# fdrmrc/fictitious_domain_AL_preconditioners

Measured on AMD Instinct MI355X. Metric: FGMRES iterations/sec to 1e-8 residual, 3D Stokes-immersed (AL-preconditioned), higher is better.
Workload: dtype f64

## Files before the change

### fictitious_domain_al_preconditioners_amd/csrc/alfd.hip

```cpp

#include <hip/hip_runtime.h>
#include <rccl/rccl.h>

#include <algorithm>
#include <atomic>
#include <chrono>
#include <cmath>
#include <cstdio>
#include <cstdlib>
#include <cstring>
#include <memory>
#include <climits>
#include <condition_variable>
#include <functional>
#include <mutex>
#include <string>
#include <thread>
#include <unordered_set>
#include <vector>

#include "alfd/alfd.h"
#include "kernels.hpp"
#include "kernels_vs.hpp"

// ... 91 lines not shown
  std::vector<int64_t> rp;
  std::vector<int32_t> col;
  std::vector<double> val;
  int64_t nnz() const { return rp.empty() ? 0 : rp.back(); }
};

constexpr int kScratchSlot = ALFD_NSLOTS;

struct MlLevel {
  DevCsr A, C, Ct;
  DevCsr P, R;
  int64_t n = 0, npad = 0;
  double *dinv = nullptr;
  double lmax = 0;
  double *r = nullptr, *z = nullptr, *t = nullptr, *cd = nullptr, *cres = nullptr, *ctmp = nullptr;
  DevCsr gA, gC, gCt, gP, gR;
  bool P_global_cols = false;
  int64_t gn = 0, gnpad = 0, g_maxpiece = 0;
  std::vector<int64_t> g_offs;
  double *gdinv = nullptr, *gr = nullptr, *gz = nullptr, *gt = nullptr, *gcd = nullptr, *gcres = nullptr,
         *gctmp = nullptr, *g_send = nullptr, *g_stage = nullptr;
};

enum State { ITERATE = 0, SUCCESS = 1, FAILURE = 2 };
struct Control {
  alfd_control c;
  double initial = 0, reduced_tol = 0, last_value = 0;
  int last_step = 0;
  State check(int step, double v) {
    last_step = step;
// ... 58 lines not shown
  double *n_sc = nullptr, *n_sc_host = nullptr, *n_partial = nullptr, *n_gather = nullptr;
  int64_t mass_its = 0;
  HostCsr h_M, h_K;
  std::vector<int32_t> ml_agg[ALFD_MAX_LEVELS];
  std::vector<double> ml_wgt[ALFD_MAX_LEVELS];
  int64_t ml_ncoarse[ALFD_MAX_LEVELS] = {0, 0, 0, 0, 0, 0, 0, 0};
  HostCsr ml_P[ALFD_MAX_LEVELS];
  DevCsr ml_inv;
  struct Patch {
    bool on = false;
    int64_t m = 0, mpad = 0;
    DevCsr Ass, As, Ats, Cs, Cts;
    int32_t *S = nullptr;
    double *dinv = nullptr, *rS = nullptr, *zS = nullptr, *uS = nullptr, *eS = nullptr, *cd = nullptr,
           *cres = nullptr, *ctmp = nullptr, *rr = nullptr;
    double lmax = 0;
    bool rep = false;
    int64_t m_loc = 0, piece = 1, lam_piece = 1;
    std::vector<int64_t> soff;
    DevCsr Cts_loc, Ctg;
    double *send = nullptr, *stage = nullptr, *lam_send = nullptr, *lam_stage = nullptr, *loc = nullptr;
  } patch;
  std::vector<MlLevel> ml;
  int ml_rep_level = -1;
  bool dots_replicated = false;
  int64_t ml_rep_threshold = 300000;
  int ml_gpu_galerkin = 1;
  double *g_w = nullptr, *g_tlam = nullptr;
  std::vector<int64_t> ml_coff[ALFD_MAX_LEVELS];
  const int64_t *up_col_offsets = nullptr;
// ... 14 lines not shown
  double lambda_max = 0, lambda_min = 0;
  int64_t inner_its = 0, mp_its = 0;
  int inner_failures = 0, precond_applications = 0;
  std::vector<double> history;
  int timing = 0;
  std::vector<TimedLaunch> timed;
  double t_ms[ALFD_T_NCLASSES] = {0, 0, 0, 0};
  int64_t t_launches[ALFD_T_NCLASSES] = {0, 0, 0, 0};
  double t_bytes[ALFD_T_NCLASSES] = {0, 0, 0, 0};
  double t_fbytes[ALFD_T_NCLASSES] = {0, 0, 0, 0};
  double setup_s[ALFD_SETUP_NPHASES] = {0, 0, 0, 0, 0, 0, 0, 0};
  bool upload_since_setup = false;
  std::vector<void *> allocs;
  int spmv_stream_R = 2, spmv_stream_U = 8, spmv_nt = 0, spmv_grid_mult = 8;
  int spmv_group_R = 4, spmv_group_U = 4;
  bool vi_off = false;
  int vi_rows_R = 4, vi_rows_J = 2;
  int vi_xcd = 0;
  int vi_levels = 1;
  int vi_batched = 1;
  int win_RB_vi = 96;
  int win_vi = 1;
  int win_short_scale = 2;
  int vs_enable = 1, vs_NW = 4, vs_RB = 96, vs_xcd = 0, vs_share = 1, vs_wide = 1;
  int vs_lds_base_ok = -1;
  std::vector<int64_t> rb_ptr[ALFD_NSLOTS + 1];
  std::vector<int32_t> rb_rows[ALFD_NSLOTS + 1];
  int win_short_min_blocks = 256;
  int win_min_blocks = 256;
  int win_enable = 1, win_RB = 96, win_maxW = 4096, win_gap = 8, win_xcd = 0;
// ... 179 lines not shown
    hipEventElapsedTime(&ms, t.a, t.b);
    ctx->t_ms[t.cls] += ms;
    hipEventDestroy(t.a);
    hipEventDestroy(t.b);
  }
  ctx->timed.clear();
}

template <int L>
static void launch_spmv_L(alfd_ctx *ctx, const DevCsr &m, const double *x, double *y, int epi, double alpha,
                          const double *d, double *y2) {
  const int grid = grid_for_rows(m.n_list, L);
  const double *xh = m.halo;
#define ALFD_SPMV(EPI, SP)                                                                          \
  hipLaunchKernelGGL((spmv_kernel<L, EPI, SP>), dim3(grid), dim3(kBlock), 0, ctx->stream, m.n_list, \
                     m.rp, m.col, m.val, m.rows, x, xh, m.n_local_cols, y, alpha, d, y2)
  if (m.sparse) {
    if (epi == 0) ALFD_SPMV(0, true);
    else if (epi == 1) ALFD_SPMV(1, true);
    else if (epi == 2) ALFD_SPMV(2, true);
    else ALFD_SPMV(3, true);
  } else {
    if (epi == 0) ALFD_SPMV(0, false);
    else if (epi == 1) ALFD_SPMV(1, false);
    else if (epi == 2) ALFD_SPMV(2, false);
    else ALFD_SPMV(3, false);
  }
#undef ALFD_SPMV
}

template <int R, int U, bool NT>
static void launch_stream(alfd_ctx *ctx, const DevCsr &m, const double *x, double *y, int epi, double alpha,
                          const double *d, double *y2) {
  const int64_t nbatches = (m.nrows + R - 1) / R;
  const int grid = (int)std::max<int64_t>(1, std::min<int64_t>((nbatches + 3) / 4, 256 * ctx->spmv_grid_mult));
#define ALFD_STREAM(EPI)                                                                              \
  hipLaunchKernelGGL((spmv_stream_kernel<R, U, EPI, NT>), dim3(grid), dim3(kBlock), 0, ctx->stream,   \
                     m.nrows, m.rp, m.col, m.val, x, m.halo, m.n_local_cols, y, alpha, d, y2)
  if (epi == 0) ALFD_STREAM(0);
  else if (epi == 1) ALFD_STREAM(1);
  else if (epi == 2) ALFD_STREAM(2);
  else ALFD_STREAM(3);
#undef ALFD_STREAM
}

template <bool NT>
static bool launch_stream_RU(alfd_ctx *ctx, const DevCsr &m, const double *x, double *y, int epi,
                             double alpha, const double *d, double *y2) {
  const int R = ctx->spmv_stream_R, U = ctx->spmv_stream_U;
#define ALFD_RU(RR, UU) \
  if (R == RR && U == UU) return launch_stream<RR, UU, NT>(ctx, m, x, y, epi, alpha, d, y2), true
  ALFD_RU(2, 2); ALFD_RU(2, 4); ALFD_RU(4, 2); ALFD_RU(4, 4); ALFD_RU(4, 8); ALFD_RU(8, 4); ALFD_RU(8, 8);
  ALFD_RU(1, 4); ALFD_RU(2, 8); ALFD_RU(8, 2);
#undef ALFD_RU
  return false;
}

// ... 111 lines not shown
  ALFD_RU(1, 4); ALFD_RU(2, 4); ALFD_RU(2, 8); ALFD_RU(4, 2); ALFD_RU(4, 4); ALFD_RU(4, 8); ALFD_RU(8, 4);
  ALFD_RU(1, 8); ALFD_RU(1, 16); ALFD_RU(2, 16);
#undef ALFD_RU
  return false;
}


template <int L>
static void launch_vss(alfd_ctx *ctx, const DevCsr &m, const double *x, double *y, int epi, double alpha,
                       const double *d, double *y2) {
  const DevCsr::Vs &v = m.vs;
  const size_t lds = (size_t)kVsWinOff + (size_t)v.maxW * sizeof(double);
#define ALFD_VSS(EPI, TAG)                                                                                          \
  hipLaunchKernelGGL((spmv_vss_kernel<L, EPI, TAG>), dim3((unsigned)v.nb), dim3(256), lds, ctx->stream, v.stream, \
                     v.sb, v.tab, v.cnt, v.stride, v.seg_begin, v.blkW, v.seg_col, v.seg_off, v.doff, v.dn, v.dict, \
                     x, m.halo, m.n_local_cols, y, alpha, d, y2)
  if (m.tag == 0) {
    if (epi == 0) ALFD_VSS(0, 0);
    else if (epi == 1) ALFD_VSS(1, 0);
    else if (epi == 2) ALFD_VSS(2, 0);
    else ALFD_VSS(3, 0);
  } else {
    if (epi == 0) ALFD_VSS(0, 1);
    else if (epi == 1) ALFD_VSS(1, 1);
    else if (epi == 2) ALFD_VSS(2, 1);
    else ALFD_VSS(3, 1);
  }
#undef ALFD_VSS
}

static bool launch_vs(alfd_ctx *ctx, const DevCsr &m, const double *x, double *y, int epi, double alpha,
                      const double *d, double *y2, int64_t first_block = 0, int64_t n_blocks = -1) {
  const DevCsr::Vs &v = m.vs;
  if (ctx->vs_lds_base_ok < 0) {
    uint32_t *probe = nullptr, base = 1;
    if (hipMalloc((void **)&probe, sizeof(uint32_t)) == hipSuccess) {
      hipLaunchKernelGGL(vs_lds_base_probe_kernel, dim3(1), dim3(64), 4096, ctx->stream, probe);
      hipMemcpyAsync(&base, probe, sizeof(uint32_t), hipMemcpyDeviceToHost, ctx->stream);
      hipStreamSynchronize(ctx->stream);
      hipFree(probe);
// ... 35 lines not shown
  } while (0)
  if (NW == 8) ALFD_VS_E(8);
  else if (NW == 2) ALFD_VS_E(2);
  else ALFD_VS_E(4);
#undef ALFD_VS_E
#undef ALFD_VS
#undef ALFD_VS_ARGS
  return true;
}

static int halo_exchange(alfd_ctx *ctx, DevCsr &m, const double *x, hipStream_t st = nullptr);
static int spmv_launch_local(alfd_ctx *ctx, DevCsr &m, const double *x, double *y, int epi, double alpha, const double *d,
                             double *y2);

static int spmv_m(alfd_ctx *ctx, DevCsr &m, int cls, const double *x, double *y, int epi, double alpha = 0.0,
                  const double *d = nullptr, double *y2 = nullptr) {
  if (!m.present) return ctx->err = "matrix not set", ALFD_E_NOT_SETUP;
  const bool exchange = ctx->nranks > 1 && !m.rep && (ctx->local || ctx->host_alltoallv || m.n_halo > 0 || m.send_off.back() > 0);
  const bool overlap = exchange && (ctx->overlap_halo > 0 || (ctx->overlap_halo < 0 && (ctx->local || ctx->host_alltoallv))) && ctx->xstream && m.vs.on && m.vs.L == 64 && ctx->vs_enable && !ctx->vi_off &&
                       m.vs.nb_interior > 0 && !m.sparse && m.n_list > 0;
  if (overlap) {
    Timer tm(ctx, cls, m.algorithmic_bytes(), m.streamed_bytes(true, true));
    HIPC(hipEventRecord(ctx->ev_x, ctx->stream));
    if (!launch_vs(ctx, m, x, y, epi, alpha, d, y2, 0, m.vs.nb_interior)) return ctx->err = "batch-major launch failed", ALFD_E_HIP;
    HIPC(hipStreamWaitEvent(ctx->xstream, ctx->ev_x, 0));
    RC(halo_exchange(ctx, m, x, ctx->xstream));
    HIPC(hipEventRecord(ctx->ev_halo, ctx->xstream));
    HIPC(hipStreamWaitEvent(ctx->stream, ctx->ev_halo, 0));
    launch_vs(ctx, m, x, y, epi, alpha, d, y2, m.vs.nb_interior, m.vs.nb - m.vs.nb_interior);
    HIPC(hipGetLastError());
    return ALFD_OK;
  }
  if (exchange) RC(halo_exchange(ctx, m, x));
  if (m.sparse && epi != 1) {
    HIPC(hipMemsetAsync(y, 0, m.nrows * sizeof(double), ctx->stream));
    if (epi == 3) HIPC(hipMemsetAsync(y2, 0, m.nrows * sizeof(double), ctx->stream));
  }
  if (m.n_list == 0) return ALFD_OK;
  Timer tm(ctx, cls, m.algorithmic_bytes(), m.streamed_bytes(!ctx->vi_off, ctx->vs_enable != 0 && !ctx->vi_off));
  return spmv_launch_local(ctx, m, x, y, epi, alpha, d, y2);
}

static int spmv_launch_local(alfd_ctx *ctx, DevCsr &m, const double *x, double *y, int epi, double alpha, const double *d,
                             double *y2) {
  if (m.vs.on && ctx->vs_enable && !ctx->vi_off && launch_vs(ctx, m, x, y, epi, alpha, d, y2)) {
    HIPC(hipGetLastError());
    return ALFD_OK;
  }
  if (m.win && launch_window_RU(ctx, m, x, y, epi, alpha, d, y2)) {
    HIPC(hipGetLastError());
    return ALFD_OK;
  }
  if (m.L == 64 && !m.sparse && ctx->spmv_stream_R > 0) {
    const bool ok = ctx->spmv_nt ? launch_stream_RU<true>(ctx, m, x, y, epi, alpha, d, y2)
                                 : launch_stream_RU<false>(ctx, m, x, y, epi, alpha, d, y2);
    if (ok) {
      HIPC(hipGetLastError());
      return ALFD_OK;
    }
  }
  switch (m.L) {
    case 4: launch_spmv_L<4>(ctx, m, x, y, epi, alpha, d, y2); break;
    case 8: launch_spmv_L<8>(ctx, m, x, y, epi, alpha, d, y2); break;
    case 16: launch_spmv_L<16>(ctx, m, x, y, epi, alpha, d, y2); break;
    case 32: launch_spmv_L<32>(ctx, m, x, y, epi, alpha, d, y2); break;
    default: launch_spmv_L<64>(ctx, m, x, y, epi, alpha, d, y2); break;
  }
  HIPC(hipGetLastError());
  return ALFD_OK;
}

static int pick_short_row_format(alfd_ctx *ctx, DevCsr &m) {
  if (!m.vs.on || m.vs.L == 64 || m.nnz < 20000000 || ctx->vi_off || !ctx->vs_enable || m.sparse) return ALFD_OK;
  double *x = nullptr, *y = nullptr;
  const int64_t nx = std::max<int64_t>(ctx->nranks > 1 && !m.rep ? m.n_local_cols : m.ncols, 1);
  HIPC(hipMalloc((void **)&x, nx * sizeof(double)));
  HIPC(hipMalloc((void **)&y, std::max<int64_t>(m.nrows, 1) * sizeof(double)));
  HIPC(hipMemsetAsync(x, 0, nx * sizeof(double), ctx->stream));
  hipEvent_t e0, e1;
  HIPC(hipEventCreate(&e0));
  HIPC(hipEventCreate(&e1));
  float t[2] = {0.f, 0.f};
  bool ok = true;
  for (int f = 0; f < 2 && ok; ++f) {
// ... 2385 lines not shown

static int upload_matrix(alfd_ctx *ctx, int slot, int64_t nrows, int64_t ncols, const int64_t *rp,
                         const int32_t *col, const double *val);
static int upload_level(alfd_ctx *ctx, DevCsr &dst, const HostCsr &h) {
  static const int32_t no_col = 0;
  static const double no_val = 0;
  RC(upload_matrix(ctx, kScratchSlot, h.nrows, h.ncols, h.rp.data(), h.col.empty() ? &no_col : h.col.data(),
                   h.val.empty() ? &no_val : h.val.data()));
  csr_free(dst);
  dst = std::move(ctx->mat[kScratchSlot]);
  ctx->mat[kScratchSlot] = DevCsr();
  dst.tag = 1;
  return ALFD_OK;
}

static int level_op(alfd_ctx *ctx, int l, const double *x, double *y) {
  if (l == 0) return op_apply(ctx, OP_AUG, x, y);
  MlLevel &L = ctx->ml[l];
  RC(spmv_m(ctx, L.A, ALFD_T_SPMV_OTHER, x, y, 0));
  if (ctx->cfg.aug_assembled) return ALFD_OK;
  RC(spmv_m(ctx, L.C, ALFD_T_SPMV_OTHER, x, ctx->t_lam, 2, 0.0, ctx->diag[ALFD_INVW]));
  return spmv_m(ctx, L.Ct, ALFD_T_SPMV_OTHER, ctx->t_lam, y, 1, ctx->cfg.gamma);
}

static int level_cheb(alfd_ctx *ctx, int l, int degree, double ratio, const double *r, double *z) {
  MlLevel &L = ctx->ml[l];
  const double lmax = L.lmax, lmin = lmax / ratio;
  const double theta = 0.5 * (lmax + lmin), delta = 0.5 * (lmax - lmin);
  const double sigma = theta / delta;
  double rho = 1.0 / sigma;
  VEC_LAUNCH(cheb_init_kernel, L.npad, degree > 1 ? 40 : 32, 1.0 / theta, L.dinv, r, L.cd, z, L.cres,
             degree > 1 ? 1 : 0);
  for (int j = 1; j < degree; ++j) {
    RC(level_op(ctx, l, L.cd, L.ctmp));
    const double rho_new = 1.0 / (2.0 * sigma - rho);
    const double c1 = rho_new * rho, c2 = 2.0 * rho_new / delta;
    VEC_LAUNCH(cheb_step_kernel, L.npad, 64, c1, c2, L.dinv, L.ctmp, L.cres, L.cd, z);
    rho = rho_new;
  }
  HIPC(hipGetLastError());
  return ALFD_OK;
}

static int level_op_rep(alfd_ctx *ctx, int l, const double *x, double *y) {
  MlLevel &L = ctx->ml[l];
  RC(spmv_m(ctx, L.gA, ALFD_T_SPMV_OTHER, x, y, 0));
  if (ctx->cfg.aug_assembled) return ALFD_OK;
  RC(spmv_m(ctx, L.gC, ALFD_T_SPMV_OTHER, x, ctx->g_tlam, 2, 0.0, ctx->g_w));
  return spmv_m(ctx, L.gCt, ALFD_T_SPMV_OTHER, ctx->g_tlam, y, 1, ctx->cfg.gamma);
}

static int level_cheb_rep(alfd_ctx *ctx, int l, int degree, double ratio, const double *r, double *z) {
  MlLevel &L = ctx->ml[l];
  const double lmax = L.lmax, lmin = lmax / ratio;
  const double theta = 0.5 * (lmax + lmin), delta = 0.5 * (lmax - lmin);
  const double sigma = theta / delta;
  double rho = 1.0 / sigma;
  VEC_LAUNCH(cheb_init_kernel, L.gnpad, degree > 1 ? 40 : 32, 1.0 / theta, L.gdinv, r, L.gcd, z, L.gcres,
             degree > 1 ? 1 : 0);
  for (int j = 1; j < degree; ++j) {
    RC(level_op_rep(ctx, l, L.gcd, L.gctmp));
    const double rho_new = 1.0 / (2.0 * sigma - rho);
    const double c1 = rho_new * rho, c2 = 2.0 * rho_new / delta;
    VEC_LAUNCH(cheb_step_kernel, L.gnpad, 64, c1, c2, L.gdinv, L.gctmp, L.gcres, L.gcd, z);
    rho = rho_new;
  }
  HIPC(hipGetLastError());
  return ALFD_OK;
}

static int ml_cycle_rep(alfd_ctx *ctx, int l, const double *r, double *z) {
  const alfd_config &c = ctx->cfg;
  const int last = (int)ctx->ml.size() - 1;
  if (l == last) {
    if (ctx->ml_inv.present) return spmv_m(ctx, ctx->ml_inv, ALFD_T_SPMV_OTHER, r, z, 0);
    return level_cheb_rep(ctx, l, c.ml_coarse_degree, c.ml_coarse_ratio, r, z);
  }
  MlLevel &L = ctx->ml[l], &N = ctx->ml[l + 1];
  const int sdeg = l > 0 && c.ml_smooth_degree_coarse > 0 ? c.ml_smooth_degree_coarse : c.ml_smooth_degree;
  RC(level_cheb_rep(ctx, l, sdeg, c.ml_smooth_ratio, r, z));
  RC(level_op_rep(ctx, l, z, L.gt));
  VEC_LAUNCH(sub_from_kernel, L.gnpad, 24, r, L.gt);
  RC(spmv_m(ctx, N.gR, ALFD_T_SPMV_OTHER, L.gt, N.gr, 0));
  RC(ml_cycle_rep(ctx, l + 1, N.gr, N.gz));
  RC(spmv_m(ctx, N.gP, ALFD_T_SPMV_OTHER, N.gz, z, 1, 1.0));
  RC(level_op_rep(ctx, l, z, L.gt));
  VEC_LAUNCH(sub_from_kernel, L.gnpad, 24, r, L.gt);
  RC(level_cheb_rep(ctx, l, sdeg, c.ml_smooth_ratio, L.gt, L.gr));
  VEC_LAUNCH(axpy_kernel, L.gnpad, 24, (const double *)nullptr, 0, 1.0, L.gr, z);
  HIPC(hipGetLastError());
  return ALFD_OK;
}

static int ml_cycle(alfd_ctx *ctx, int l, const double *r, double *z) {
  const alfd_config &c = ctx->cfg;
  const int last = (int)ctx->ml.size() - 1;
  if (l == last) {
    if (ctx->ml_inv.present) return spmv_m(ctx, ctx->ml_inv, ALFD_T_SPMV_OTHER, r, z, 0);
    return level_cheb(ctx, l, c.ml_coarse_degree, c.ml_coarse_ratio, r, z);
  }
  MlLevel &L = ctx->ml[l], &N = ctx->ml[l + 1];
  const int sdeg = l > 0 && c.ml_smooth_degree_coarse > 0 ? c.ml_smooth_degree_coarse : c.ml_smooth_degree;
  RC(level_cheb(ctx, l, sdeg, c.ml_smooth_ratio, r, z));
  RC(level_op(ctx, l, z, L.t));
  VEC_LAUNCH(sub_from_kernel, L.npad, 24, r, L.t);
  RC(spmv_m(ctx, N.R, ALFD_T_SPMV_OTHER, L.t, N.r, 0));
  if (l + 1 == ctx->ml_rep_level) {
    HIPC(hipMemcpyAsync(N.g_send, N.r, N.n * sizeof(double), hipMemcpyDeviceToDevice, ctx->stream));
    RC(comm_allgather(ctx, N.g_send, N.g_stage, (size_t)N.g_maxpiece * sizeof(double)));
    for (int p = 0; p < ctx->nranks; ++p) {
      const int64_t np = N.g_offs[p + 1] - N.g_offs[p];
      if (np > 0)
        HIPC(hipMemcpyAsync(N.gr + N.g_offs[p], N.g_stage + (int64_t)p * N.g_maxpiece, np * sizeof(double),
                            hipMemcpyDeviceToDevice, ctx->stream));
    }
    RC(ml_cycle_rep(ctx, l + 1, N.gr, N.gz));
    RC(spmv_m(ctx, N.P, ALFD_T_SPMV_OTHER, N.P_global_cols ? N.gz : N.gz + N.g_offs[ctx->rank], z, 1, 1.0));
  } else {
    RC(ml_cycle(ctx, l + 1, N.r, N.z));
    RC(spmv_m(ctx, N.P, ALFD_T_SPMV_OTHER, N.z, z, 1, 1.0));
  }
  RC(level_op(ctx, l, z, L.t));
  VEC_LAUNCH(sub_from_kernel, L.npad, 24, r, L.t);
  RC(level_cheb(ctx, l, sdeg, c.ml_smooth_ratio, L.t, L.r));
  VEC_LAUNCH(axpy_kernel, L.npad, 24, (const double *)nullptr, 0, 1.0, L.r, z);
  HIPC(hipGetLastError());
  return ALFD_OK;
}

static int ws_alloc_zero(alfd_ctx *ctx, double **p, int64_t count);

static int patch_op(alfd_ctx *ctx, const double *x, double *y) {
  alfd_ctx::Patch &Q = ctx->patch;
  RC(spmv_m(ctx, Q.Ass, ALFD_T_SPMV_OTHER, x, y, 0));
  if (ctx->cfg.aug_assembled) return ALFD_OK;
  double *t = Q.rep ? ctx->g_tlam : ctx->t_lam;
  const double *w = Q.rep ? ctx->g_w : ctx->diag[ALFD_INVW];
  RC(spmv_m(ctx, Q.Cs, ALFD_T_SPMV_OTHER, x, t, 2, 0.0, w));
  return spmv_m(ctx, Q.Cts, ALFD_T_SPMV_OTHER, t, y, 1, ctx->cfg.gamma);
}

static int patch_cheb(alfd_ctx *ctx, const double *r, double *z) {
  alfd_ctx::Patch &Q = ctx->patch;
  const int degree = ctx->cfg.ml_patch_degree;
  const double lmax = Q.lmax, lmin = lmax / ctx->cfg.ml_patch_ratio;
  const double theta = 0.5 * (lmax + lmin), delta = 0.5 * (lmax - lmin);
  const double sigma = theta / delta;
  double rho = 1.0 / sigma;
  VEC_LAUNCH(cheb_init_kernel, Q.mpad, degree > 1 ? 40 : 32, 1.0 / theta, Q.dinv, r, Q.cd, z, Q.cres, degree > 1 ? 1 : 0);
  for (int j = 1; j < degree; ++j) {
    RC(patch_op(ctx, Q.cd, Q.ctmp));
    const double rho_new = 1.0 / (2.0 * sigma - rho);
    const double c1 = rho_new * rho, c2 = 2.0 * rho_new / delta;
    VEC_LAUNCH(cheb_step_kernel, Q.mpad, 64, c1, c2, Q.dinv, Q.ctmp, Q.cres, Q.cd, z);
    rho = rho_new;
  }
  HIPC(hipGetLastError());
  return ALFD_OK;
}

static int allgather_pieces(alfd_ctx *ctx, const double *mine, const std::vector<int64_t> &offs, int64_t piece, double *send,
                            double *stage, double *whole) {
  const int64_t n_me = offs[ctx->rank + 1] - offs[ctx->rank];
  if (n_me > 0) HIPC(hipMemcpyAsync(send, mine, n_me * sizeof(double), hipMemcpyDeviceToDevice, ctx->stream));
  RC(comm_allgather(ctx, send, stage, (size_t)piece * sizeof(double)));
  for (int p = 0; p < ctx->nranks; ++p) {
    const int64_t np = offs[p + 1] - offs[p];
    if (np > 0)
      HIPC(hipMemcpyAsync(whole + offs[p], stage + (int64_t)p * piece, np * sizeof(double), hipMemcpyDeviceToDevice, ctx->stream));
  }
  return ALFD_OK;
}

// ... 1624 lines not shown
  if (hipGetDeviceCount(&ndev) != hipSuccess || ndev <= 0 || device_id < 0 || device_id >= ndev)
    return ALFD_E_HIP;
  if (hipSetDevice(device_id) != hipSuccess) return ALFD_E_HIP;
  alfd_ctx *ctx = new alfd_ctx;
  ctx->device = device_id;
  if (hipStreamCreateWithFlags(&ctx->xstream, hipStreamNonBlocking) != hipSuccess ||
      hipEventCreateWithFlags(&ctx->ev_x, hipEventDisableTiming) != hipSuccess ||
      hipEventCreateWithFlags(&ctx->ev_halo, hipEventDisableTiming) != hipSuccess)
    ctx->xstream = nullptr;
  if (const char *e = std::getenv("ALFD_SPMV_OVERLAP_HALO")) ctx->overlap_halo = std::atoi(e);
  if (hipStreamCreateWithFlags(&ctx->stream, hipStreamNonBlocking) != hipSuccess) {
    delete ctx;
    return ALFD_E_HIP;
  }
  alfd_default_config(&ctx->cfg, ALFD_AL_STOKES);
  if (const char *e = std::getenv("ALFD_SPMV_STREAM_R")) ctx->spmv_stream_R = std::atoi(e);
  if (const char *e = std::getenv("ALFD_SPMV_STREAM_U")) ctx->spmv_stream_U = std::atoi(e);
  if (const char *e = std::getenv("ALFD_SPMV_NT")) ctx->spmv_nt = std::atoi(e);
  if (const char *e = std::getenv("ALFD_SPMV_GRID")) ctx->spmv_grid_mult = std::max(1, std::atoi(e));
  if (const char *e = std::getenv("ALFD_SPMV_WINDOW")) ctx->win_enable = std::atoi(e);
  if (const char *e = std::getenv("ALFD_SPMV_WINDOW_RB")) ctx->win_RB = std::max(4, std::atoi(e));
  if (const char *e = std::getenv("ALFD_SPMV_WINDOW_MIN_BLOCKS")) ctx->win_min_blocks = std::max(1, std::atoi(e));
  if (const char *e = std::getenv("ALFD_SPMV_WINDOW_SHORT_MIN_BLOCKS")) ctx->win_short_min_blocks = std::max(1, std::atoi(e));
  if (const char *e = std::getenv("ALFD_SPMV_WINDOW_MAXW")) ctx->win_maxW = std::min(16384, std::max(256, std::atoi(e)));
  if (const char *e = std::getenv("ALFD_ML_REPLICATE")) ctx->ml_rep_threshold = std::atoll(e);
  if (const char *e = std::getenv("ALFD_ML_GPU_GALERKIN")) ctx->ml_gpu_galerkin = std::atoi(e);
  if (const char *e = std::getenv("ALFD_SPMV_VI_LEVELS")) ctx->vi_levels = std::atoi(e);
  if (const char *e = std::getenv("ALFD_SPMV_BATCH_MAJOR")) ctx->vs_enable = std::atoi(e);
  if (const char *e = std::getenv("ALFD_SPMV_BATCH_MAJOR_ROWS")) ctx->vs_RB = std::max(4, std::min(kVsMaxRows, std::atoi(e)));
  if (const char *e = std::getenv("ALFD_SPMV_VI_XCD")) ctx->vi_xcd = std::atoi(e);
// ... 1015 lines not shown
  CHECK_CTX();
  size_t f = 0, t = 0;
  HIPC(hipMemGetInfo(&f, &t));
  if (free_bytes) *free_bytes = (int64_t)f;
  if (total_bytes) *total_bytes = (int64_t)t;
  return ALFD_OK;
}

int alfd_set_tunable(alfd_ctx_t ctx, const char *name, int value) {
  if (!ctx || !name) return ALFD_E_INVALID;
  if (std::strcmp(name, "value_index") == 0) {
    ctx->vi_off = value == 0;
    if (value == 0) RC(ensure_window_plans(ctx));
    return ALFD_OK;
  }
  if (std::strcmp(name, "batch_major") == 0) {
    ctx->vs_enable = value != 0;
    if (value == 0) RC(ensure_window_plans(ctx));
    return ALFD_OK;
  }
  if (std::strcmp(name, "batch_major_share") == 0) {
    ctx->vs_share = value != 0;
    return ALFD_OK;
  }
  if (std::strcmp(name, "batch_major_wide") == 0) {
    ctx->vs_wide = value != 0;
    return ALFD_OK;
  }
  if (std::strcmp(name, "batch_major_waves") == 0) {
    if (value != 2 && value != 4 && value != 8) return ctx->err = "batch_major_waves: 2, 4 or 8", ALFD_E_INVALID;
// ... 59 lines not shown
```

### fictitious_domain_al_preconditioners_amd/csrc/kernels.hpp

```cpp
#pragma once
#include <hip/hip_runtime.h>
#include <stdint.h>

namespace alfd {

constexpr int kBlock = 256;
constexpr int64_t kChunk = 4096;
constexpr int kMaxBasis = 64;

__device__ __forceinline__ double dpp_xor_mov(double v, int which) {
  int lo = __double2loint(v), hi = __double2hiint(v), rl, rh;
  if (which == 8) {
    rl = __builtin_amdgcn_update_dpp(0, lo, 0x128, 0xf, 0xf, true);
    rh = __builtin_amdgcn_update_dpp(0, hi, 0x128, 0xf, 0xf, true);
  } else if (which == 4) {
    rl = __builtin_amdgcn_update_dpp(0, lo, 0x104, 0xf, 0x5, false);
    rl = __builtin_amdgcn_update_dpp(rl, lo, 0x114, 0xf, 0xa, false);
    rh = __builtin_amdgcn_update_dpp(0, hi, 0x104, 0xf, 0x5, false);
    rh = __builtin_amdgcn_update_dpp(rh, hi, 0x114, 0xf, 0xa, false);
  } else if (which == 2) {
    rl = __builtin_amdgcn_update_dpp(0, lo, 0x4E, 0xf, 0xf, true);
    rh = __builtin_amdgcn_update_dpp(0, hi, 0x4E, 0xf, 0xf, true);
  } else {
    rl = __builtin_amdgcn_update_dpp(0, lo, 0xB1, 0xf, 0xf, true);
// ... 110 lines not shown
__device__ __forceinline__ double reduce_rows2(double a0, double a1) {
  swap32(a0, a1);
  double p = a0 + a1, q = p;
  swap16(p, q);
  return row16_tree(p + q);
}

__device__ __forceinline__ double block_reduce_256(double v, double *lds4) {
  v = group_reduce<64>(v);
  const int wave = threadIdx.x >> 6;
  if ((threadIdx.x & 63) == 0) lds4[wave] = v;
  __syncthreads();
  return (lds4[0] + lds4[1]) + (lds4[2] + lds4[3]);
}

template <int L, int EPI, bool SPARSE>
__global__ __launch_bounds__(kBlock) void spmv_kernel(int64_t nrows, const int64_t *__restrict__ rp,
                                                      const int32_t *__restrict__ col,
                                                      const double *__restrict__ val,
                                                      const int32_t *__restrict__ rows,
                                                      const double *__restrict__ x,
                                                      const double *__restrict__ x_halo, int32_t n_local,
                                                      double *__restrict__ y, double alpha,
                                                      const double *__restrict__ d,
                                                      double *__restrict__ y2) {
  constexpr int RPB = kBlock / L;
  const int lane = threadIdx.x % L;
  const int sub = threadIdx.x / L;
  const int64_t ngroups = (nrows + RPB - 1) / RPB;
  for (int64_t g = blockIdx.x; g < ngroups; g += gridDim.x) {
    const int64_t r = g * RPB + sub;
    if (r < nrows) {
      const int64_t k0 = rp[r], k1 = rp[r + 1];
      double acc = 0.0;
      for (int64_t k = k0 + lane; k < k1; k += L) {
        const int32_t c = col[k];
        const double xv = (c < n_local) ? x[c] : x_halo[c - n_local];
        acc = fma(val[k], xv, acc);
      }
      acc = group_reduce<L>(acc);
      if (lane == 0) {
        const int64_t ro = SPARSE ? (int64_t)rows[r] : r;
        if (EPI == 0)
          y[ro] = acc;
        else if (EPI == 1)
          y[ro] = fma(alpha, acc, y[ro]);
        else if (EPI == 2)
          y[ro] = d[ro] * acc;
        else {
          y[ro] = acc;
          y2[ro] = d[ro] * acc;
        }
      }
    }
  }
}

template <int R, int U, int EPI, bool NT>
__global__ __launch_bounds__(kBlock) void spmv_stream_kernel(
    int64_t nrows, const int64_t *__restrict__ rp, const int32_t *__restrict__ col,
    const double *__restrict__ val, const double *__restrict__ x, const double *__restrict__ x_halo,
    int32_t n_local, double *__restrict__ y, double alpha, const double *__restrict__ d,
    double *__restrict__ y2) {
  const int lane = threadIdx.x & 63;
  const int wave = __builtin_amdgcn_readfirstlane(threadIdx.x >> 6);
  const int64_t nbatches = (nrows + R - 1) / R;
  for (int64_t b = (int64_t)blockIdx.x * 4 + wave; b < nbatches; b += (int64_t)gridDim.x * 4) {
    const int64_t r0 = b * R;
    int64_t kb[R + 1];
#pragma unroll
    for (int i = 0; i <= R; ++i) kb[i] = rp[r0 + i < nrows ? r0 + i : nrows];
    const int64_t k_begin = kb[0];
    const int32_t n_batch = (int32_t)(kb[R] - k_begin);
    int32_t rel[R + 1];
#pragma unroll
    for (int i = 0; i <= R; ++i) rel[i] = (int32_t)(kb[i] - k_begin);
    double acc[R];
#pragma unroll
// ... 31 lines not shown
    }
#pragma unroll
    for (int i = 0; i < R; ++i) {
      const int64_t r = r0 + i;
      if (r < nrows) {
        const int dsh = rel[i] & 63;
        double s = __shfl(acc[i], (lane + dsh) & 63, 64);
        s = group_reduce<64>(s);
        if (lane == 0) {
          if (EPI == 0)
            y[r] = s;
          else if (EPI == 1)
            y[r] = fma(alpha, s, y[r]);
          else if (EPI == 2)
            y[r] = d[r] * s;
          else {
            y[r] = s;
            y2[r] = d[r] * s;
          }
        }
      }
    }
  }
}

template <int R, int U, int EPI, int TAG = 0>
__global__ __launch_bounds__(kBlock) void spmv_window_kernel(
    int64_t nrows, int32_t RB, const int64_t *__restrict__ rp, const int32_t *__restrict__ col,
    const uint16_t *__restrict__ lcol, const double *__restrict__ val,
    const int32_t *__restrict__ blk_seg_begin, const int32_t *__restrict__ blk_W,
// ... 1115 lines not shown
```

### fictitious_domain_al_preconditioners_amd/csrc/kernels_vs.hpp

```cpp
#pragma once

namespace alfd {

constexpr int kVsMaxDict = 512;
constexpr int kVsDictOff = 0;
constexpr int kVsWinOff = kVsMaxDict * 8;
constexpr int kVsMaxRows = 250;
template <int WD>
struct VsFmt {
  static constexpr uint32_t kColMask = WD ? 0x3ff8u : 0x7ff8u;
  static constexpr int kDictShift = WD ? 11 : 12;
  static constexpr uint32_t kDictMask = WD ? 0x1ff8u : 0xff8u;
  static constexpr int kWinOff = WD ? 8192 : 4096;
  static constexpr int kCodeShift = WD ? 14 : 15;
  static constexpr int kMaxDict = WD ? 1024 : 512;
  static constexpr int kMaxSlots = WD ? 2048 : 4096;
};
constexpr int kVsMaxLen = 384;

__device__ __forceinline__ uint32_t vs_off(uint32_t d) { return d & 0xfffffu; }
__device__ __forceinline__ int32_t vs_len(uint32_t d) { return (int32_t)((d >> 20) & 0x1ffu); }
__device__ __forceinline__ int vs_cls(uint32_t d) { return (int)((d >> 29) & 7u); }

__device__ __forceinline__ double vs_lds_f64(uint32_t byte_off) {
// ... 260 lines not shown
    }
    hv1 = hv2;
    if (bi + NW < nbatch && (int32_t)n1 < 0) vs_shared_fetch(n0, sbase, lane, w);
    hv2 = hdr_load(bi + 2 * NW);
    if (mstep) store(sres, rid, (lane & (mstep - 1)) == 0);
  }
}

template <int L, int EPI, int TAG>
__global__ __launch_bounds__(256) __attribute__((amdgpu_waves_per_eu(8, 8))) void spmv_vss_kernel(
    const uint8_t *__restrict__ stream, const int64_t *__restrict__ sb, const uint64_t *__restrict__ tab,
    const int32_t *__restrict__ cnt, int32_t stride, const int32_t *__restrict__ blk_seg_begin,
    const int32_t *__restrict__ blk_W, const int32_t *__restrict__ seg_col, const int32_t *__restrict__ seg_off,
    const int32_t *__restrict__ blk_dict_off, const int32_t *__restrict__ blk_dict_n,
    const double *__restrict__ dict, const double *__restrict__ x, const double *__restrict__ x_halo,
    int32_t n_local, double *__restrict__ y, double alpha, const double *__restrict__ d, double *__restrict__ y2) {
  extern __shared__ double xs[];
  constexpr int G = 64 / L, W64 = 1 + 4 * G, NW = 4;
  char *sm = (char *)xs;
  double *ds = (double *)(sm + kVsDictOff);
  double *xw = (double *)(sm + kVsWinOff);
  const int lane = threadIdx.x & 63;
  const int wave = __builtin_amdgcn_readfirstlane(threadIdx.x >> 6);
  const int l = lane & (L - 1), g = lane / L;
  const int64_t b = blockIdx.x;
  const int32_t nbatch = cnt[b];
  const uint8_t *sbase = stream + sb[b];
  {
    const int32_t nd = blk_dict_n[b];
    for (int t = threadIdx.x; t < nd; t += 64 * NW) ds[t] = dict[blk_dict_off[b] + t];
    const int32_t W = blk_W[b];
// ... 65 lines not shown
        if (L * j + l < len) {
          asm volatile("");
#pragma unroll
          for (int q = 0; q < 4; ++q) acc[q] = fma(v, xv[q], acc[q]);
        }
      }
    }
    auto store = [&](double s, int32_t r, bool writer) {
      if (writer && r >= 0) {
        if (EPI == 0)
          y[r] = s;
        else if (EPI == 1)
          y[r] = fma(alpha, s, y[r]);
        else if (EPI == 2)
          y[r] = d[r] * s;
        else {
          y[r] = s;
          y2[r] = d[r] * s;
        }
      }
    };
    const bool w8 = (lane & 7) == 0, h8 = (lane & 8) != 0;
    if (L == 32) {
      swap16(acc[0], acc[1]);
      double u = acc[0] + acc[1];
      swap16(acc[2], acc[3]);
      double w = acc[2] + acc[3];
      u = u + dpp_xor_mov(u, 8);
      w = w + dpp_xor_mov(w, 8);
      double t = h8 ? w : u;
// ... 39 lines not shown
```

Baseline: 14.38.

## Fuse Chebyshev smoother updates and residuals into SpMV epilogues

Adds a FusedEpi epilogue to the SpMV kernels so each Chebyshev step, the initial residual-plus-init, and the multigrid residual computation happen inside the A-SpMV instead of as separate vector kernels. The Ct·t contribution is computed first into a separate buffer and added in the epilogue with gamma. The aim is to remove separate vector launches and the extra passes over the ctmp/res/z vectors, and to fold the post-smoothing residual into the first smoother step. It also unifies the level, replicated and patch smoother code into one path. The cost is more register pressure and more per-row traffic inside the SpMV epilogue, plus an extra buffer when the augmented operator is not assembled.

```diff
diff --git a/fictitious_domain_al_preconditioners_amd/csrc/alfd.hip b/fictitious_domain_al_preconditioners_amd/csrc/alfd.hip
--- a/fictitious_domain_al_preconditioners_amd/csrc/alfd.hip
+++ b/fictitious_domain_al_preconditioners_amd/csrc/alfd.hip
@@ -129,6 +129,7 @@
   double *dinv = nullptr;
   double lmax = 0;
   double *r = nullptr, *z = nullptr, *t = nullptr, *cd = nullptr, *cres = nullptr, *ctmp = nullptr;
+  double *cu = nullptr, *gcu = nullptr;
   DevCsr gA, gC, gCt, gP, gR;
   bool P_global_cols = false;
   int64_t gn = 0, gnpad = 0, g_maxpiece = 0;
@@ -217,6 +218,7 @@
     int32_t *S = nullptr;
     double *dinv = nullptr, *rS = nullptr, *zS = nullptr, *uS = nullptr, *eS = nullptr, *cd = nullptr,
            *cres = nullptr, *ctmp = nullptr, *rr = nullptr;
+    double *cu = nullptr;
     double lmax = 0;
     bool rep = false;
     int64_t m_loc = 0, piece = 1, lam_piece = 1;
@@ -261,6 +263,9 @@
   std::vector<void *> allocs;
   int spmv_stream_R = 2, spmv_stream_U = 8, spmv_nt = 0, spmv_grid_mult = 8;
   int spmv_group_R = 4, spmv_group_U = 4;
+  int fused_smoother = 1;
+  FusedEpi fe{};
+  double fe_bytes = 0;
   bool vi_off = false;
   int vi_rows_R = 4, vi_rows_J = 2;
   int vi_xcd = 0;
@@ -470,7 +475,7 @@
   const double *xh = m.halo;
 #define ALFD_SPMV(EPI, SP)                                                                          \
   hipLaunchKernelGGL((spmv_kernel<L, EPI, SP>), dim3(grid), dim3(kBlock), 0, ctx->stream, m.n_list, \
-                     m.rp, m.col, m.val, m.rows, x, xh, m.n_local_cols, y, alpha, d, y2)
+                     m.rp, m.col, m.val, m.rows, x, xh, m.n_local_cols, y, alpha, d, y2, ctx->fe)
   if (m.sparse) {
     if (epi == 0) ALFD_SPMV(0, true);
     else if (epi == 1) ALFD_SPMV(1, true);
@@ -480,10 +485,14 @@
     if (epi == 0) ALFD_SPMV(0, false);
     else if (epi == 1) ALFD_SPMV(1, false);
     else if (epi == 2) ALFD_SPMV(2, false);
+    else if (epi == 4) ALFD_SPMV(4, false);
+    else if (epi == 5) ALFD_SPMV(5, false);
     else ALFD_SPMV(3, false);
   }
 #undef ALFD_SPMV
 }
+
+static constexpr bool fused_stream_shape(int R, int U, bool NT) { return R == 2 && U == 8 && !NT; }
 
 template <int R, int U, bool NT>
 static void launch_stream(alfd_ctx *ctx, const DevCsr &m, const double *x, double *y, int epi, double alpha,
@@ -492,11 +501,15 @@
   const int grid = (int)std::max<int64_t>(1, std::min<int64_t>((nbatches + 3) / 4, 256 * ctx->spmv_grid_mult));
 #define ALFD_STREAM(EPI)                                                                              \
   hipLaunchKernelGGL((spmv_stream_kernel<R, U, EPI, NT>), dim3(grid), dim3(kBlock), 0, ctx->stream,   \
-                     m.nrows, m.rp, m.col, m.val, x, m.halo, m.n_local_cols, y, alpha, d, y2)
+                     m.nrows, m.rp, m.col, m.val, x, m.halo, m.n_local_cols, y, alpha, d, y2, ctx->fe)
   if (epi == 0) ALFD_STREAM(0);
   else if (epi == 1) ALFD_STREAM(1);
   else if (epi == 2) ALFD_STREAM(2);
-  else ALFD_STREAM(3);
+  else if (epi < 4) ALFD_STREAM(3);
+  else if constexpr (fused_stream_shape(R, U, NT)) {
+    if (epi == 4) ALFD_STREAM(4);
+    else ALFD_STREAM(5);
+  }
 #undef ALFD_STREAM
 }
 
@@ -638,16 +651,20 @@
 #define ALFD_VSS(EPI, TAG)                                                                                          \
   hipLaunchKernelGGL((spmv_vss_kernel<L, EPI, TAG>), dim3((unsigned)v.nb), dim3(256), lds, ctx->stream, v.stream, \
                      v.sb, v.tab, v.cnt, v.stride, v.seg_begin, v.blkW, v.seg_col, v.seg_off, v.doff, v.dn, v.dict, \
-                     x, m.halo, m.n_local_cols, y, alpha, d, y2)
+                     x, m.halo, m.n_local_cols, y, alpha, d, y2, ctx->fe)
   if (m.tag == 0) {
     if (epi == 0) ALFD_VSS(0, 0);
     else if (epi == 1) ALFD_VSS(1, 0);
     else if (epi == 2) ALFD_VSS(2, 0);
+    else if (epi == 4) ALFD_VSS(4, 0);
+    else if (epi == 5) ALFD_VSS(5, 0);
     else ALFD_VSS(3, 0);
   } else {
     if (epi == 0) ALFD_VSS(0, 1);
     else if (epi == 1) ALFD_VSS(1, 1);
     else if (epi == 2) ALFD_VSS(2, 1);
+    else if (epi == 4) ALFD_VSS(4, 1);
+    else if (epi == 5) ALFD_VSS(5, 1);
     else ALFD_VSS(3, 1);
   }
 #undef ALFD_VSS
@@ -713,13 +730,14 @@
                              double *y2);
 
 static int spmv_m(alfd_ctx *ctx, DevCsr &m, int cls, const double *x, double *y, int epi, double alpha = 0.0,
-                  const double *d = nullptr, double *y2 = nullptr) {
+                  const double *d = nullptr, double *y2 = nullptr, bool listed_only = false) {
   if (!m.present) return ctx->err = "matrix not set", ALFD_E_NOT_SETUP;
   const bool exchange = ctx->nranks > 1 && !m.rep && (ctx->local || ctx->host_alltoallv || m.n_halo > 0 || m.send_off.back() > 0);
   const bool overlap = exchange && (ctx->overlap_halo > 0 || (ctx->overlap_halo < 0 && (ctx->local || ctx->host_alltoallv))) && ctx->xstream && m.vs.on && m.vs.L == 64 && ctx->vs_enable && !ctx->vi_off &&
                        m.vs.nb_interior > 0 && !m.sparse && m.n_list > 0;
   if (overlap) {
-    Timer tm(ctx, cls, m.algorithmic_bytes(), m.streamed_bytes(true, true));
+    const double eb = epi >= 4 ? ctx->fe_bytes : 0.0;
+    Timer tm(ctx, cls, m.algorithmic_bytes() + eb, m.streamed_bytes(true, true) + eb);
     HIPC(hipEventRecord(ctx->ev_x, ctx->stream));
     if (!launch_vs(ctx, m, x, y, epi, alpha, d, y2, 0, m.vs.nb_interior)) return ctx->err = "batch-major launch failed", ALFD_E_HIP;
     HIPC(hipStreamWaitEvent(ctx->xstream, ctx->ev_x, 0));
@@ -731,12 +749,13 @@
     return ALFD_OK;
   }
   if (exchange) RC(halo_exchange(ctx, m, x));
-  if (m.sparse && epi != 1) {
+  if (m.sparse && epi != 1 && !listed_only) {
     HIPC(hipMemsetAsync(y, 0, m.nrows * sizeof(double), ctx->stream));
     if (epi == 3) HIPC(hipMemsetAsync(y2, 0, m.nrows * sizeof(double), ctx->stream));
   }
   if (m.n_list == 0) return ALFD_OK;
-  Timer tm(ctx, cls, m.algorithmic_bytes(), m.streamed_bytes(!ctx->vi_off, ctx->vs_enable != 0 && !ctx->vi_off));
+  const double eb = epi >= 4 ? ctx->fe_bytes : 0.0;
+  Timer tm(ctx, cls, m.algorithmic_bytes() + eb, m.streamed_bytes(!ctx->vi_off, ctx->vs_enable != 0 && !ctx->vi_off) + eb);
   return spmv_launch_local(ctx, m, x, y, epi, alpha, d, y2);
 }
 
@@ -767,6 +786,18 @@
   }
   HIPC(hipGetLastError());
   return ALFD_OK;
+}
+
+static bool fused_spmv_ok(const alfd_ctx *ctx, const DevCsr &m) {
+  if (!m.present || m.sparse || m.nrows <= 0 || m.n_list != m.nrows) return false;
+  if (m.vs.on && ctx->vs_enable && !ctx->vi_off) {
+    if (ctx->vs_lds_base_ok != 1) return false;
+    return m.vs.L == 32 || m.vs.L == 16 || m.vs.L == 8;
+  }
+  if (m.win) return false;
+  if (m.L == 64 && ctx->spmv_stream_R > 0)
+    return fused_stream_shape(ctx->spmv_stream_R, ctx->spmv_stream_U, ctx->spmv_nt != 0);
+  return m.L == 4 || m.L == 8 || m.L == 16 || m.L == 32 || m.L == 64;
 }
 
 static int pick_short_row_format(alfd_ctx *ctx, DevCsr &m) {
@@ -3182,59 +3213,144 @@
   return ALFD_OK;
 }
 
-static int level_op(alfd_ctx *ctx, int l, const double *x, double *y) {
-  if (l == 0) return op_apply(ctx, OP_AUG, x, y);
+static int ws_alloc_zero(alfd_ctx *ctx, double **p, int64_t count);
+
+struct AugOp {
+  DevCsr *A, *C, *Ct;
+  int cls;
+  const double *w;
+  double *t;
+  int64_t npad;
+  const double *dinv;
+  double *cd, *cres, *ctmp;
+  double **cu;
+};
+
+static AugOp level_aug(alfd_ctx *ctx, int l) {
   MlLevel &L = ctx->ml[l];
-  RC(spmv_m(ctx, L.A, ALFD_T_SPMV_OTHER, x, y, 0));
+  if (l == 0)
+    return {&ctx->mat[ALFD_A], &ctx->mat[ALFD_C], &ctx->mat[ALFD_CT], ALFD_T_SPMV_A, ctx->diag[ALFD_INVW], ctx->t_lam,
+            L.npad, L.dinv, L.cd, L.cres, L.ctmp, &L.cu};
+  return {&L.A, &L.C, &L.Ct, ALFD_T_SPMV_OTHER, ctx->diag[ALFD_INVW], ctx->t_lam, L.npad, L.dinv, L.cd, L.cres, L.ctmp,
+          &L.cu};
+}
+
+static AugOp level_aug_rep(alfd_ctx *ctx, int l) {
+  MlLevel &L = ctx->ml[l];
+  return {&L.gA, &L.gC, &L.gCt, ALFD_T_SPMV_OTHER, ctx->g_w, ctx->g_tlam, L.gnpad, L.gdinv, L.gcd, L.gcres, L.gctmp,
+          &L.gcu};
+}
+
+static AugOp patch_aug(alfd_ctx *ctx) {
+  alfd_ctx::Patch &Q = ctx->patch;
+  return {&Q.Ass, &Q.Cs, &Q.Cts, ALFD_T_SPMV_OTHER, Q.rep ? ctx->g_w : ctx->diag[ALFD_INVW], Q.rep ? ctx->g_tlam : ctx->t_lam,
+          Q.mpad, Q.dinv, Q.cd, Q.cres, Q.ctmp, &Q.cu};
+}
+
+static int aug_apply(alfd_ctx *ctx, const AugOp &op, const double *x, double *y) {
+  RC(spmv_m(ctx, *op.A, op.cls, x, y, 0));
   if (ctx->cfg.aug_assembled) return ALFD_OK;
-  RC(spmv_m(ctx, L.C, ALFD_T_SPMV_OTHER, x, ctx->t_lam, 2, 0.0, ctx->diag[ALFD_INVW]));
-  return spmv_m(ctx, L.Ct, ALFD_T_SPMV_OTHER, ctx->t_lam, y, 1, ctx->cfg.gamma);
-}
-
-static int level_cheb(alfd_ctx *ctx, int l, int degree, double ratio, const double *r, double *z) {
-  MlLevel &L = ctx->ml[l];
-  const double lmax = L.lmax, lmin = lmax / ratio;
+  RC(spmv_m(ctx, *op.C, ALFD_T_SPMV_OTHER, x, op.t, 2, 0.0, op.w));
+  return spmv_m(ctx, *op.Ct, ALFD_T_SPMV_OTHER, op.t, y, 1, ctx->cfg.gamma);
+}
+
+static bool aug_fused_ok(const alfd_ctx *ctx, const AugOp &op) {
+  return ctx->fused_smoother && fused_spmv_ok(ctx, *op.A);
+}
+
+static int aug_fused(alfd_ctx *ctx, const AugOp &op, const double *x, int epi, FusedEpi fe, double row_bytes) {
+  fe.has_u = ctx->cfg.aug_assembled ? 0 : 1;
+  fe.gamma = ctx->cfg.gamma;
+  fe.u = nullptr;
+  if (fe.has_u) {
+    if (!*op.cu) RC(ws_alloc_zero(ctx, op.cu, op.npad));
+    RC(spmv_m(ctx, *op.C, ALFD_T_SPMV_OTHER, x, op.t, 2, 0.0, op.w));
+    RC(spmv_m(ctx, *op.Ct, ALFD_T_SPMV_OTHER, op.t, *op.cu, 0, 0.0, nullptr, nullptr, true));
+    fe.u = *op.cu;
+    row_bytes += 8;
+  }
+  ctx->fe = fe;
+  ctx->fe_bytes = row_bytes * (double)op.A->nrows;
+  const int rc = spmv_m(ctx, *op.A, op.cls, x, nullptr, epi);
+  ctx->fe = FusedEpi{};
+  ctx->fe_bytes = 0;
+  return rc;
+}
+
+static int aug_residual(alfd_ctx *ctx, const AugOp &op, const double *b, const double *x, double *t) {
+  if (aug_fused_ok(ctx, op)) {
+    FusedEpi fe{};
+    fe.b = b;
+    fe.res = t;
+    return aug_fused(ctx, op, x, 5, fe, 16);
+  }
+  RC(aug_apply(ctx, op, x, t));
+  VEC_LAUNCH(sub_from_kernel, op.npad, 24, b, t);
+  HIPC(hipGetLastError());
+  return ALFD_OK;
+}
+
+static int aug_cheb(alfd_ctx *ctx, const AugOp &op, int degree, double lmax, double ratio, const double *r,
+                    const double *xr, double *t, double *z) {
+  const double lmin = lmax / ratio;
   const double theta = 0.5 * (lmax + lmin), delta = 0.5 * (lmax - lmin);
   const double sigma = theta / delta;
   double rho = 1.0 / sigma;
-  VEC_LAUNCH(cheb_init_kernel, L.npad, degree > 1 ? 40 : 32, 1.0 / theta, L.dinv, r, L.cd, z, L.cres,
-             degree > 1 ? 1 : 0);
+  const bool fused = aug_fused_ok(ctx, op);
+  if (fused && xr) {
+    FusedEpi fe{};
+    fe.b = r;
+    fe.res = degree > 1 ? op.cres : nullptr;
+    fe.dinv = op.dinv;
+    fe.d_out = op.cd;
+    fe.z = z;
+    fe.inv_theta = 1.0 / theta;
+    fe.init = 1;
+    RC(aug_fused(ctx, op, xr, 5, fe, degree > 1 ? 40 : 32));
+  } else {
+    if (xr) {
+      RC(aug_apply(ctx, op, xr, t));
+      VEC_LAUNCH(sub_from_kernel, op.npad, 24, r, t);
+      r = t;
+    }
+    VEC_LAUNCH(cheb_init_kernel, op.npad, degree > 1 ? 40 : 32, 1.0 / theta, op.dinv, r, op.cd, z, op.cres,
+               degree > 1 ? 1 : 0);
+  }
+  double *d = op.cd, *d2 = op.ctmp;
   for (int j = 1; j < degree; ++j) {
-    RC(level_op(ctx, l, L.cd, L.ctmp));
     const double rho_new = 1.0 / (2.0 * sigma - rho);
     const double c1 = rho_new * rho, c2 = 2.0 * rho_new / delta;
-    VEC_LAUNCH(cheb_step_kernel, L.npad, 64, c1, c2, L.dinv, L.ctmp, L.cres, L.cd, z);
+    if (fused) {
+      FusedEpi fe{};
+      fe.dinv = op.dinv;
+      fe.res = op.cres;
+      fe.d_in = d;
+      fe.d_out = d2;
+      fe.z = z;
+      fe.c1 = c1;
+      fe.c2 = c2;
+      RC(aug_fused(ctx, op, d, 4, fe, 56));
+      std::swap(d, d2);
+    } else {
+      RC(aug_apply(ctx, op, op.cd, op.ctmp));
+      VEC_LAUNCH(cheb_step_kernel, op.npad, 64, c1, c2, op.dinv, op.ctmp, op.cres, op.cd, z);
+    }
     rho = rho_new;
   }
   HIPC(hipGetLastError());
   return ALFD_OK;
 }
 
+static int level_op(alfd_ctx *ctx, int l, const double *x, double *y) { return aug_apply(ctx, level_aug(ctx, l), x, y); }
 static int level_op_rep(alfd_ctx *ctx, int l, const double *x, double *y) {
-  MlLevel &L = ctx->ml[l];
-  RC(spmv_m(ctx, L.gA, ALFD_T_SPMV_OTHER, x, y, 0));
-  if (ctx->cfg.aug_assembled) return ALFD_OK;
-  RC(spmv_m(ctx, L.gC, ALFD_T_SPMV_OTHER, x, ctx->g_tlam, 2, 0.0, ctx->g_w));
-  return spmv_m(ctx, L.gCt, ALFD_T_SPMV_OTHER, ctx->g_tlam, y, 1, ctx->cfg.gamma);
-}
-
+  return aug_apply(ctx, level_aug_rep(ctx, l), x, y);
+}
+
+static int level_cheb(alfd_ctx *ctx, int l, int degree, double ratio, const double *r, double *z) {
+  return aug_cheb(ctx, level_aug(ctx, l), degree, ctx->ml[l].lmax, ratio, r, nullptr, nullptr, z);
+}
 static int level_cheb_rep(alfd_ctx *ctx, int l, int degree, double ratio, const double *r, double *z) {
-  MlLevel &L = ctx->ml[l];
-  const double lmax = L.lmax, lmin = lmax / ratio;
-  const double theta = 0.5 * (lmax + lmin), delta = 0.5 * (lmax - lmin);
-  const double sigma = theta / delta;
-  double rho = 1.0 / sigma;
-  VEC_LAUNCH(cheb_init_kernel, L.gnpad, degree > 1 ? 40 : 32, 1.0 / theta, L.gdinv, r, L.gcd, z, L.gcres,
-             degree > 1 ? 1 : 0);
-  for (int j = 1; j < degree; ++j) {
-    RC(level_op_rep(ctx, l, L.gcd, L.gctmp));
-    const double rho_new = 1.0 / (2.0 * sigma - rho);
-    const double c1 = rho_new * rho, c2 = 2.0 * rho_new / delta;
-    VEC_LAUNCH(cheb_step_kernel, L.gnpad, 64, c1, c2, L.gdinv, L.gctmp, L.gcres, L.gcd, z);
-    rho = rho_new;
-  }
-  HIPC(hipGetLastError());
-  return ALFD_OK;
+  return aug_cheb(ctx, level_aug_rep(ctx, l), degree, ctx->ml[l].lmax, ratio, r, nullptr, nullptr, z);
 }
 
 static int ml_cycle_rep(alfd_ctx *ctx, int l, const double *r, double *z) {
@@ -3245,16 +3361,14 @@
     return level_cheb_rep(ctx, l, c.ml_coarse_degree, c.ml_coarse_ratio, r, z);
   }
   MlLevel &L = ctx->ml[l], &N = ctx->ml[l + 1];
+  const AugOp op = level_aug_rep(ctx, l);
   const int sdeg = l > 0 && c.ml_smooth_degree_coarse > 0 ? c.ml_smooth_degree_coarse : c.ml_smooth_degree;
   RC(level_cheb_rep(ctx, l, sdeg, c.ml_smooth_ratio, r, z));
-  RC(level_op_rep(ctx, l, z, L.gt));
-  VEC_LAUNCH(sub_from_kernel, L.gnpad, 24, r, L.gt);
+  RC(aug_residual(ctx, op, r, z, L.gt));
   RC(spmv_m(ctx, N.gR, ALFD_T_SPMV_OTHER, L.gt, N.gr, 0));
   RC(ml_cycle_rep(ctx, l + 1, N.gr, N.gz));
   RC(spmv_m(ctx, N.gP, ALFD_T_SPMV_OTHER, N.gz, z, 1, 1.0));
-  RC(level_op_rep(ctx, l, z, L.gt));
-  VEC_LAUNCH(sub_from_kernel, L.gnpad, 24, r, L.gt);
-  RC(level_cheb_rep(ctx, l, sdeg, c.ml_smooth_ratio, L.gt, L.gr));
+  RC(aug_cheb(ctx, op, sdeg, L.lmax, c.ml_smooth_ratio, r, z, L.gt, L.gr));
   VEC_LAUNCH(axpy_kernel, L.gnpad, 24, (const double *)nullptr, 0, 1.0, L.gr, z);
   HIPC(hipGetLastError());
   return ALFD_OK;
@@ -3268,10 +3382,10 @@
     return level_cheb(ctx, l, c.ml_coarse_degree, c.ml_coarse_ratio, r, z);
   }
   MlLevel &L = ctx->ml[l], &N = ctx->ml[l + 1];
+  const AugOp op = level_aug(ctx, l);
   const int sdeg = l > 0 && c.ml_smooth_degree_coarse > 0 ? c.ml_smooth_degree_coarse : c.ml_smooth_degree;
   RC(level_cheb(ctx, l, sdeg, c.ml_smooth_ratio, r, z));
-  RC(level_op(ctx, l, z, L.t));
-  VEC_LAUNCH(sub_from_kernel, L.npad, 24, r, L.t);
+  RC(aug_residual(ctx, op, r, z, L.t));
   RC(spmv_m(ctx, N.R, ALFD_T_SPMV_OTHER, L.t, N.r, 0));
   if (l + 1 == ctx->ml_rep_level) {
     HIPC(hipMemcpyAsync(N.g_send, N.r, N.n * sizeof(double), hipMemcpyDeviceToDevice, ctx->stream));
@@ -3288,43 +3402,17 @@
     RC(ml_cycle(ctx, l + 1, N.r, N.z));
     RC(spmv_m(ctx, N.P, ALFD_T_SPMV_OTHER, N.z, z, 1, 1.0));
   }
-  RC(level_op(ctx, l, z, L.t));
-  VEC_LAUNCH(sub_from_kernel, L.npad, 24, r, L.t);
-  RC(level_cheb(ctx, l, sdeg, c.ml_smooth_ratio, L.t, L.r));
+  RC(aug_cheb(ctx, op, sdeg, L.lmax, c.ml_smooth_ratio, r, z, L.t, L.r));
   VEC_LAUNCH(axpy_kernel, L.npad, 24, (const double *)nullptr, 0, 1.0, L.r, z);
   HIPC(hipGetLastError());
   return ALFD_OK;
 }
 
-static int ws_alloc_zero(alfd_ctx *ctx, double **p, int64_t count);
-
-static int patch_op(alfd_ctx *ctx, const double *x, double *y) {
-  alfd_ctx::Patch &Q = ctx->patch;
-  RC(spmv_m(ctx, Q.Ass, ALFD_T_SPMV_OTHER, x, y, 0));
-  if (ctx->cfg.aug_assembled) return ALFD_OK;
-  double *t = Q.rep ? ctx->g_tlam : ctx->t_lam;
-  const double *w = Q.rep ? ctx->g_w : ctx->diag[ALFD_INVW];
-  RC(spmv_m(ctx, Q.Cs, ALFD_T_SPMV_OTHER, x, t, 2, 0.0, w));
-  return spmv_m(ctx, Q.Cts, ALFD_T_SPMV_OTHER, t, y, 1, ctx->cfg.gamma);
-}
+static int patch_op(alfd_ctx *ctx, const double *x, double *y) { return aug_apply(ctx, patch_aug(ctx), x, y); }
 
 static int patch_cheb(alfd_ctx *ctx, const double *r, double *z) {
-  alfd_ctx::Patch &Q = ctx->patch;
-  const int degree = ctx->cfg.ml_patch_degree;
-  const double lmax = Q.lmax, lmin = lmax / ctx->cfg.ml_patch_ratio;
-  const double theta = 0.5 * (lmax + lmin), delta = 0.5 * (lmax - lmin);
-  const double sigma = theta / delta;
-  double rho = 1.0 / sigma;
-  VEC_LAUNCH(cheb_init_kernel, Q.mpad, degree > 1 ? 40 : 32, 1.0 / theta, Q.dinv, r, Q.cd, z, Q.cres, degree > 1 ? 1 : 0);
-  for (int j = 1; j < degree; ++j) {
-    RC(patch_op(ctx, Q.cd, Q.ctmp));
-    const double rho_new = 1.0 / (2.0 * sigma - rho);
-    const double c1 = rho_new * rho, c2 = 2.0 * rho_new / delta;
-    VEC_LAUNCH(cheb_step_kernel, Q.mpad, 64, c1, c2, Q.dinv, Q.ctmp, Q.cres, Q.cd, z);
-    rho = rho_new;
-  }
-  HIPC(hipGetLastError());
-  return ALFD_OK;
+  return aug_cheb(ctx, patch_aug(ctx), ctx->cfg.ml_patch_degree, ctx->patch.lmax, ctx->cfg.ml_patch_ratio, r, nullptr,
+                  nullptr, z);
 }
 
 static int allgather_pieces(alfd_ctx *ctx, const double *mine, const std::vector<int64_t> &offs, int64_t piece, double *send,
@@ -4979,6 +5067,7 @@
     return ALFD_E_HIP;
   }
   alfd_default_config(&ctx->cfg, ALFD_AL_STOKES);
+  if (const char *e = std::getenv("ALFD_FUSED_SMOOTHER")) ctx->fused_smoother = std::atoi(e) != 0;
   if (const char *e = std::getenv("ALFD_SPMV_STREAM_R")) ctx->spmv_stream_R = std::atoi(e);
   if (const char *e = std::getenv("ALFD_SPMV_STREAM_U")) ctx->spmv_stream_U = std::atoi(e);
   if (const char *e = std::getenv("ALFD_SPMV_NT")) ctx->spmv_nt = std::atoi(e);
@@ -6024,6 +6113,10 @@
     if (value == 0) RC(ensure_window_plans(ctx));
     return ALFD_OK;
   }
+  if (std::strcmp(name, "fused_smoother") == 0) {
+    ctx->fused_smoother = value != 0;
+    return ALFD_OK;
+  }
   if (std::strcmp(name, "batch_major") == 0) {
     ctx->vs_enable = value != 0;
     if (value == 0) RC(ensure_window_plans(ctx));
diff --git a/fictitious_domain_al_preconditioners_amd/csrc/kernels.hpp b/fictitious_domain_al_preconditioners_amd/csrc/kernels.hpp
--- a/fictitious_domain_al_preconditioners_amd/csrc/kernels.hpp
+++ b/fictitious_domain_al_preconditioners_amd/csrc/kernels.hpp
@@ -148,6 +148,35 @@
   return (lds4[0] + lds4[1]) + (lds4[2] + lds4[3]);
 }
 
+struct FusedEpi {
+  const double *dinv, *b, *u;
+  double *res;
+  const double *d_in;
+  double *d_out, *z;
+  double c1, c2, gamma, inv_theta;
+  int has_u, init;
+};
+
+template <int EPI>
+__device__ __forceinline__ void fused_epilogue(const FusedEpi &e, int64_t r, double s) {
+  const double tmp = e.has_u ? fma(e.gamma, e.u[r], s) : s;
+  if (EPI == 4) {
+    const double rv = e.res[r] - tmp;
+    const double dd = fma(e.c1, e.d_in[r], e.c2 * (e.dinv[r] * rv));
+    e.res[r] = rv;
+    e.d_out[r] = dd;
+    e.z[r] = e.z[r] + dd;
+  } else {
+    const double t = e.b[r] - tmp;
+    if (e.res) e.res[r] = t;
+    if (e.init) {
+      const double o = e.inv_theta * (e.dinv[r] * t);
+      e.d_out[r] = o;
+      e.z[r] = o;
+    }
+  }
+}
+
 template <int L, int EPI, bool SPARSE>
 __global__ __launch_bounds__(kBlock) void spmv_kernel(int64_t nrows, const int64_t *__restrict__ rp,
                                                       const int32_t *__restrict__ col,
@@ -157,7 +186,7 @@
                                                       const double *__restrict__ x_halo, int32_t n_local,
                                                       double *__restrict__ y, double alpha,
                                                       const double *__restrict__ d,
-                                                      double *__restrict__ y2) {
+                                                      double *__restrict__ y2, const FusedEpi fe) {
   constexpr int RPB = kBlock / L;
   const int lane = threadIdx.x % L;
   const int sub = threadIdx.x / L;
@@ -181,6 +210,8 @@
           y[ro] = fma(alpha, acc, y[ro]);
         else if (EPI == 2)
           y[ro] = d[ro] * acc;
+        else if (EPI >= 4)
+          fused_epilogue<EPI>(fe, ro, acc);
         else {
           y[ro] = acc;
           y2[ro] = d[ro] * acc;
@@ -195,7 +226,7 @@
     int64_t nrows, const int64_t *__restrict__ rp, const int32_t *__restrict__ col,
     const double *__restrict__ val, const double *__restrict__ x, const double *__restrict__ x_halo,
     int32_t n_local, double *__restrict__ y, double alpha, const double *__restrict__ d,
-    double *__restrict__ y2) {
+    double *__restrict__ y2, const FusedEpi fe) {
   const int lane = threadIdx.x & 63;
   const int wave = __builtin_amdgcn_readfirstlane(threadIdx.x >> 6);
   const int64_t nbatches = (nrows + R - 1) / R;
@@ -257,6 +288,8 @@
             y[r] = fma(alpha, s, y[r]);
           else if (EPI == 2)
             y[r] = d[r] * s;
+          else if (EPI >= 4)
+            fused_epilogue<EPI>(fe, r, s);
           else {
             y[r] = s;
             y2[r] = d[r] * s;
diff --git a/fictitious_domain_al_preconditioners_amd/csrc/kernels_vs.hpp b/fictitious_domain_al_preconditioners_amd/csrc/kernels_vs.hpp
--- a/fictitious_domain_al_preconditioners_amd/csrc/kernels_vs.hpp
+++ b/fictitious_domain_al_preconditioners_amd/csrc/kernels_vs.hpp
@@ -298,7 +298,8 @@
     const int32_t *__restrict__ blk_W, const int32_t *__restrict__ seg_col, const int32_t *__restrict__ seg_off,
     const int32_t *__restrict__ blk_dict_off, const int32_t *__restrict__ blk_dict_n,
     const double *__restrict__ dict, const double *__restrict__ x, const double *__restrict__ x_halo,
-    int32_t n_local, double *__restrict__ y, double alpha, const double *__restrict__ d, double *__restrict__ y2) {
+    int32_t n_local, double *__restrict__ y, double alpha, const double *__restrict__ d, double *__restrict__ y2,
+    const FusedEpi fe) {
   extern __shared__ double xs[];
   constexpr int G = 64 / L, W64 = 1 + 4 * G, NW = 4;
   char *sm = (char *)xs;
@@ -394,6 +395,8 @@
           y[r] = fma(alpha, s, y[r]);
         else if (EPI == 2)
           y[r] = d[r] * s;
+        else if (EPI >= 4)
+          fused_epilogue<EPI>(fe, r, s);
         else {
           y[r] = s;
           y2[r] = d[r] * s;
```

Result: no change. 14.43, median of 3 (+0.3%).
